# Villen-Lab/pyAscore

Hardware: AMD Instinct MI355X
Metric: PSMs/sec (Ascore.score) at 1/2/4/8 MI355X + HBM-roofline % (higher is better)
Workload: dtype f32/f64 scalar + i32 counts

## Files before the change

### pyascore_amd/csrc/common.h

```cpp
#ifndef PYA_COMMON_H
#define PYA_COMMON_H

#include <stdint.h>

#define PYA_WAVE 64
#define PYA_NTOP 10
#define PYA_NTOP_MAX 16
#define PYA_NO_MATCH 15
#define PYA_TABLE_PAD 4
#define PYA_MAX_L 64
#define PYA_MAX_TYPES 8
#define PYA_MAX_NL 8
#define PYA_FAST_NL 4
#define PYA_MAX_UNIQ_WIDE 48
#define PYA_MAX_NL_CANDS 44
#define PYA_MAX_UNIQ 16
#define PYA_MAX_LIST 2048
#define PYA_MAX_LUT_N 4096
#define PYA_MAX_PUSHED 128

#define PYA_ST_OK 0
#define PYA_ST_NO_BINS 1
#define PYA_ST_TOO_MANY_BINS 2
#define PYA_ST_LUT_RANGE 3
// ... 117 lines not shown
```

### pyascore_amd/csrc/fused_core.hip.h

```cpp
#ifndef PYA_FUSED_CORE_H
#define PYA_FUSED_CORE_H
#include "score_core.hip.h"
#include "localize_core.hip.h"

#define FUSED_ROUND 3

struct FusedLds {
    uint16_t *grid;
    uint4 *cum_lut;
    PeakEntry *peaks;
    float2 *resd;
    uint8_t *rkl;
    uint32_t *rec;
    float *wsl;
    float *mass_l;
    uint32_t *flag_l;
    uint8_t *site_pos;
    float *selm;
    unsigned char *sort_raw;
    PushedEntry *pushed;
    unsigned long long *site_alt;
    uint32_t *site_max, *site_tie, *n_pushed;
    float *sc;
    uint32_t *c_tr, *c_cnt;
// ... 8 lines not shown
__host__ __device__ static inline size_t fused_align16(size_t v) { return (v + 15) & ~(size_t)15; }
__host__ __device__ static inline size_t fused_sort_bytes(uint32_t n) {
    if (n <= 64) return ((size_t)n * 10 + 15) & ~(size_t)15;
    return (((size_t)n * 6 + 15) & ~(size_t)15) + ((size_t)n / 64 + 2) * 16 + 2 * 128 * 2;
}
__host__ __device__ static inline uint32_t fused_site_cap(uint32_t push_cap) {
    const uint32_t v = (push_cap + 3u) & ~3u;
    return v > 64u ? 64u : (v < 4u ? 4u : v);
}
__host__ __device__ static inline size_t fused_post_bytes(uint32_t n_cap, uint32_t push_cap, uint32_t ent_cap, uint32_t ndir,
                                                          bool multi_z) {
    return fused_align16(fused_sort_bytes(n_cap)) + (size_t)push_cap * 16 + (size_t)fused_site_cap(push_cap) * 16 + 16 +
           (size_t)(1 + FUSED_ROUND) * 40 + (size_t)FUSED_ROUND * (16 * ndir + 4 + 4) + 16 + 64 +
           (multi_z ? fused_align16((size_t)FUSED_ROUND * ndir * 2 * ent_cap * 4) +
                          fused_align16((size_t)FUSED_ROUND * ndir * 2 * ent_cap)
                    : 0);
}
__host__ __device__ static inline size_t fused_walk_bytes(uint32_t cap) {
    return 16 * 16 + ((size_t)cap + PYA_TABLE_PAD) * 8;
}
__host__ __device__ static inline size_t fused_kept_bytes(uint32_t n_cap, uint32_t stride, uint32_t pos_cap, uint32_t ent_cap,
                                                          uint32_t ndir) {
    return fused_align16(((size_t)pos_cap + 1) * 8) + fused_align16((size_t)ent_cap * stride) + (size_t)n_cap * 16 + 256 +
           fused_align16((size_t)pos_cap + 1) + (size_t)(1 + FUSED_ROUND) * ndir * ent_cap * 4;
}
__host__ __device__ static inline size_t fused_lds_bytes(uint32_t cap, uint32_t n_cap, uint32_t stride, uint32_t pos_cap,
                                                         uint32_t ent_cap, uint32_t push_cap, uint32_t ndir, bool multi_z) {
    const size_t walk = fused_walk_bytes(cap), post = fused_post_bytes(n_cap, push_cap, ent_cap, ndir, multi_z);
    return PYA_GRID_CELLS * 2 + fused_align16(walk > post ? walk : post) +
           fused_kept_bytes(n_cap, stride, pos_cap, ent_cap, ndir) + 16;
}

DEV FusedLds fused_carve(unsigned char *raw, uint32_t cap, uint32_t n_cap, uint32_t stride, uint32_t pos_cap,
                         uint32_t ent_cap, uint32_t push_cap, uint32_t ndir, bool multi_z) {
    FusedLds f;
    f.grid = (uint16_t *)raw;
    size_t o = PYA_GRID_CELLS * 2;
    f.cum_lut = (uint4 *)(raw + o);
    f.peaks = (PeakEntry *)(raw + o + 16 * 16);
// ... 14 lines not shown
    q += (size_t)(1 + FUSED_ROUND) * 40;
    f.c_tr = (uint32_t *)(raw + q);
    q += (size_t)FUSED_ROUND * ndir * 8;
    f.c_cnt = (uint32_t *)(raw + q);
    q += (size_t)FUSED_ROUND * ndir * 8;
    f.c_depth = (int32_t *)(raw + q);
    q += FUSED_ROUND * 4;
    f.c_site = (uint32_t *)(raw + q);
    q += FUSED_ROUND * 4;
    f.bad_tasks = (uint32_t *)(raw + q);
    q += 16;
    f.t_lo = (uint32_t *)(raw + q);
    f.t_off = f.t_lo + 8;
    q += 64;
    f.srt_v = (float *)(raw + q);
    q += fused_align16((size_t)FUSED_ROUND * ndir * 2 * ent_cap * 4);
    f.srt_h = (uint8_t *)(raw + q);
    const size_t walk = fused_walk_bytes(cap), post = fused_post_bytes(n_cap, push_cap, ent_cap, ndir, multi_z);
    o += fused_align16(walk > post ? walk : post);
    f.resd = (float2 *)(raw + o);
    o += fused_align16(((size_t)pos_cap + 1) * 8);
    f.rkl = (uint8_t *)(raw + o);
    o += fused_align16((size_t)ent_cap * stride);
    f.rec = (uint32_t *)(raw + o);
    o += (size_t)n_cap * 12;
    f.wsl = (float *)(raw + o);
    o += (size_t)n_cap * 4;
    f.mass_l = (float *)(raw + o);
    f.flag_l = (uint32_t *)(raw + o + 128);
    f.site_pos = (uint8_t *)(raw + o + 256);
    f.selm = (float *)(raw + o + 256 + fused_align16((size_t)pos_cap + 1));
    return f;
}


template <bool BZ>
DEV void walk_record_steps(const float2 *&rp, int rstride, StepBits &bits, float &running, const uint4 *lut, CumCounts &cum,
                           const PeakTable &tab, int zmax, double A, double B, uint8_t *&ro, int stride, int count) {
    for (int i = 0; i < count; i++, rp += rstride) {
        const float2 mm = *rp;
        running = (bits.next() ? mm.y : mm.x) + running;
        const double m = BZ ? (double)running + A : ((double)running + A) - B;
        for (int z = 1; z <= zmax; z++, ro += stride) {
            const Look k = look4(tab, charge_mz(m, z));
            int rk = k.best;
            if (k.more()) rk = look_rest(tab, k);
// ... 701 lines not shown
```

### pyascore_amd/csrc/host_internal.h

```cpp
#ifndef PYA_HOST_INTERNAL_H
#define PYA_HOST_INTERNAL_H
#include <hip/hip_runtime_api.h>

#include <algorithm>
#include <atomic>
#include <cmath>
#include <cstdarg>
#include <cstdio>
#include <cstdlib>
#include <chrono>
#include <cstring>
#include <condition_variable>
#include <map>
#include <memory>
#include <mutex>
#include <string>
#include <thread>
#include <unordered_map>
#include <vector>

#include "../../include/pyascore_hip.h"
#include "common.h"

void pya_score_table_extend(float mz_error, uint32_t n_top, uint32_t n_to, std::vector<float> &lut,
// ... 37 lines not shown
int pya_launch_score_big(const BatchDev *b, const uint32_t *d_ids, uint32_t n_ids, uint32_t cap, uint32_t pos_cap, uint32_t kc,
                         uint32_t inline_on, hipStream_t stream);
size_t pya_localize_recount_lds_bytes(uint32_t cap, uint32_t push_cap, uint32_t pos_cap, uint32_t pool_cap, uint32_t sb);
size_t pya_localize_hash_lds_bytes(uint32_t push_cap, uint32_t n_cap, uint32_t pos_cap, uint32_t sb, uint32_t vc, uint32_t hs,
                                   uint32_t pp, uint32_t max_k, uint32_t n_nl);
int pya_launch_localize_hash(const BatchDev *b, const uint32_t *d_ids, uint32_t n_ids, uint32_t push_cap, uint32_t n_cap,
                             uint32_t pos_cap, uint32_t pool_cap, uint32_t sb, uint32_t gtp, uint32_t vc, uint32_t hs, uint32_t pp,
                             uint32_t n_nl, hipStream_t stream);
int pya_launch_localize_recount(const BatchDev *b, const uint32_t *d_ids, uint32_t n_ids, uint32_t cap, uint32_t push_cap,
                                uint32_t pos_cap, uint32_t pool_cap, uint32_t sb, uint32_t gtp, uint32_t *d_redo_count, uint32_t *d_redo_ids, hipStream_t stream);
int pya_launch_score_big_list(const BatchDev *b, const uint32_t *d_count, const uint32_t *d_ids, uint32_t n_max, uint32_t cap,
                              uint32_t pos_cap, uint32_t kc, hipStream_t stream);
uint32_t pya_big_inline_max(void);
size_t pya_fused_lds_bytes(uint32_t cap, uint32_t n_cap, uint32_t stride, uint32_t pos_cap, uint32_t ent_cap, uint32_t push_cap,
                           uint32_t both, uint32_t multi_z);
int pya_launch_fused(const BatchDev *b, const uint32_t *d_ids, uint32_t n_ids, uint32_t cap, uint32_t n_cap,
                     uint32_t stride, uint32_t pos_cap, uint32_t ent_cap, uint32_t push_cap, uint32_t both,
                     uint32_t multi_z, uint32_t *d_redo_count, uint32_t *d_redo_ids, hipStream_t stream);
size_t pya_score_cnt_lds_bytes(uint32_t cap, uint32_t pos_cap, uint32_t kc, uint32_t k_cap, uint32_t n_cap);
int pya_launch_score_cnt(const BatchDev *b, const uint32_t *d_ids, uint32_t n_ids, uint32_t cap, uint32_t pos_cap, uint32_t kc, uint32_t k_cap,
                         uint32_t n_cap, hipStream_t stream);
size_t pya_score_cntg_lds_bytes(uint32_t cap, uint32_t pos_cap, uint32_t k_cap, uint32_t n_cap, uint32_t nl_cap);
int pya_launch_score_cntg(const BatchDev *b, const uint32_t *d_ids, uint32_t n_ids, uint32_t cap, uint32_t pos_cap, uint32_t k_cap, uint32_t n_cap,
                          uint32_t nl_cap, hipStream_t stream);
size_t pya_bin_global_scratch_bytes(uint32_t cap);
int pya_launch_bin_global(const BatchDev *b, const uint32_t *d_ids, uint32_t n_ids, unsigned char *d_scratch, uint64_t stride,
                          uint32_t cap, hipStream_t stream);
size_t pya_general_lds_bytes(uint32_t l_cap, uint32_t list_cap);
size_t pya_general_scratch_bytes(uint32_t n_cap, uint32_t push_cap);
int pya_launch_general(const BatchDev *b, const uint32_t *d_ids, uint32_t n_ids, unsigned char *d_scratch, const uint64_t *d_scratch_off,
                       uint32_t l_cap, uint32_t list_cap, hipStream_t stream);
int pya_launch_general_ambiguity(const BatchDev *b, uint32_t psm, uint32_t l_cap, uint32_t list_cap, uint64_t ref_bits,
                                 uint64_t oth_bits, const float *d_scores, uint32_t n_scores, float ref_ws, float oth_ws,
// ... 92 lines not shown
        case 'N': return 114.04293f;  case 'D': return 115.02694f;  case 'Q': return 128.05858f;
        case 'K': return 128.09496f;  case 'E': return 129.04259f;  case 'M': return 131.04049f;
        case 'H': return 137.05891f;  case 'F': return 147.06841f;  case 'U': return 150.95364f;
        case 'R': return 156.10111f;  case 'Y': return 163.06333f;  case 'W': return 186.07931f;
        case 'O': return 237.14773f;
    }
    return 0.f;
}


struct Knobs {
    bool no_plain = false, no_fused = false, no_big = false, no_tiny = false, no_prefix = false, no_chunks = false;
    bool no_upload_thread = false, one_peak_class = false, peak_classes = false, one_lds_class = false;
    bool host_timing = false, stamps = false, sort_room = false, no_big_inline = false;
    bool no_loc_hash = false, no_nodes = false, no_cnt = false;
    bool no_fork = false;
    bool slow_null_stream = false;
    uint32_t debug = 0;
    int64_t plain_min = 512, big_min_n = 1024, tiny_max = 64;
    int64_t bin_select_min = 640;
    int64_t bin_select_scap = 768;
    uint32_t sort_room_max = 1024;
    int sb = -1, gtp = -1, hash_pp = -1;
    int node_cap = -1;
    double chunk_mb = 0.;
    int64_t workspace_mb = 0;
};

void read_knobs(Knobs &k);
bool set_knob(Knobs &k, const char *key, const char *value);
// ... 212 lines not shown
    DevBuf<uint32_t> d_redo3;
    DevBuf<uint32_t> d_redo;
    Bucket buckets[kNumBuckets];
    struct IdList {
        uint32_t off, n, cap, ncls;
    };
    static bool any_ids(const std::vector<IdList> &lists) {
        bool any = false;
        for (const IdList &l : lists) any = any || l.n != 0;
        return any;
    }
    std::vector<uint32_t> bin_ids, score_ids, fused_ids, big_ids;
    std::vector<IdList> bin_lists, score_lists, big_lists;
    struct FusedLaunch {
        uint32_t off, n, cap, multi_z, n_cap, stride, pos_cap, ent_cap, push_cap;
    };
    std::vector<FusedLaunch> fused_launches;
    uint32_t n_fused_total = 0;
    std::vector<uint8_t> gen;
    std::vector<uint32_t> gen_ids;
    DevBuf<uint32_t> d_gen_ids;
    DevBuf<unsigned char> d_gen_scratch;
    uint32_t gen_l_cap = 1, gen_list_cap = 1;
    std::vector<uint64_t> gen_off;
    DevBuf<uint64_t> d_gen_off;
    std::vector<uint32_t> bigbin_ids;
    DevBuf<uint32_t> d_bigbin_ids;
    DevBuf<unsigned char> d_bigbin_scratch;
    uint32_t bigbin_cap = 32;
    size_t bigbin_stride = 0;
    std::vector<uint8_t> big;
    DevBuf<uint32_t> d_big_ids;
    uint32_t big_pos_cap = 1, big_k_max = 1;
// ... 119 lines not shown
```

### pyascore_amd/csrc/host_plan.cpp

```cpp
#include "host_internal.h"

int check_psm_shape(const pya_handle *h, uint64_t i, int64_t P, int64_t L, int32_t k, int32_t z, const uint8_t *pep,
                    const uint32_t *aux_pos, int64_t n_aux, uint32_t *ns, char *msg) {
    const unsigned long long iu = i;
    auto say = [msg](int code, const char *fmt, auto... args) {
        std::snprintf(msg, kPsmMsg, fmt, args...);
        return code;
    };
    if (P <= 0) return say(PYA_ERR_PSM, "PSM %llu: empty spectrum", iu);
    if (P > PYA_MAX_PEAKS) return say(PYA_ERR_LIMIT, "PSM %llu: %lld peaks exceed the limit of %d", iu, (long long)P, PYA_MAX_PEAKS);
    if (L < 1 || L > PYA_MAX_PEPTIDE_LEN)
        return say(L < 1 ? PYA_ERR_PSM : PYA_ERR_LIMIT, "PSM %llu: peptide length %lld outside 1..%d", iu, (long long)L, PYA_MAX_PEPTIDE_LEN);
    if (k < 0) return say(PYA_ERR_PSM, "PSM %llu: negative n_of_mod", iu);
    if (z < 1 || z > PYA_MAX_CHARGE)
        return say(z < 1 ? PYA_ERR_PSM : PYA_ERR_LIMIT, "PSM %llu: max_fragment_charge %d outside 1..%d", iu, z, PYA_MAX_CHARGE);
    if (n_aux < 0) return say(PYA_ERR_ARG, "PSM %llu: aux_off is not monotone", iu);
    uint32_t cnt = 0;
    int64_t bad_j = -1, bad_a = -1;
    for (int64_t j = 0; j < L; j++) {
        if (!h->is_residue[pep[j]] && bad_j < 0) bad_j = j;
        if (h->letter_modifiable((char)pep[j], (size_t)j, (size_t)L)) cnt++;
    }
    for (int64_t a = 0; a < n_aux; a++)
        if (aux_pos[a] > (uint32_t)L && bad_a < 0) bad_a = a;
// ... 24 lines not shown
    std::vector<uint8_t> bad;
    std::vector<uint32_t> caps;
    std::vector<uint8_t> pcls;

    PlanBuild(pya_handle *h_, const pya_batch *b_, const IoReq *io_, uint32_t flags_, pya_plan *p_)
        : h(h_), b(b_), io(io_), flags(flags_), p(p_), n(b_->n_psm) {
        const DevConfig &c = h->cfg;
        const Knobs &kn = h->kn;
        has_aux = b->aux_off && b->aux_pos && b->aux_mass;
        plain_on = c.n_nl == 0 && !(flags & PYA_FLAG_KEEP) && !kn.no_plain && n >= (uint64_t)kn.plain_min;
        both_dirs = c.n_fwd > 0 && c.n_fwd < c.n_types;
        fused_on = plain_on && plain_types(c) && !kn.no_fused;
        big_on = c.n_nl == 0 && both_dirs && c.n_fwd == 1 && c.n_types == 2 && h->mz_error <= 0.49f && !kn.no_big;
        big_inline_ok = big_on && plain_on && !kn.no_big_inline;
        big_inline_max = pya_big_inline_max();
    }
};

struct Lap {
    bool on;
    std::chrono::steady_clock::time_point t0 = std::chrono::steady_clock::now();
    void operator()(const char *what) {
        if (!on) return;
        auto t1 = std::chrono::steady_clock::now();
        std::fprintf(stderr, "[pya plan] %-14s %8.3f ms\n", what, std::chrono::duration<double, std::milli>(t1 - t0).count());
        t0 = t1;
    }
};

int copy_meta(PlanBuild &B) {
// ... 240 lines not shown
            const size_t at = (size_t)(q * (double)(n - 1));
            size_t acc = 0;
            uint32_t v = 0;
            for (; v < hist.size(); v++) {
                acc += hist[v];
                if (acc > at) break;
            }
            caps.push_back((v + 31u) & ~31u);
        }
    }
    if (!caps.empty() && p->peak_cap < 2 * caps[0] && !h->kn.peak_classes) caps.clear();
    caps.push_back(p->peak_cap);
    std::sort(caps.begin(), caps.end());
    caps.erase(std::unique(caps.begin(), caps.end()), caps.end());
    const size_t nc = caps.size();
    std::vector<uint32_t> cnt_bin(nc, 0), cnt_score(nc * kNumBuckets, 0), cnt_big(nc, 0);
    B.pcls.resize(n);
    for (uint64_t i = 0; i < n; i++) {
        if (p->pre_status[i]) continue;
        const uint32_t P = (uint32_t)(p->peak_off[i + 1] - p->peak_off[i]);
        if (P > PYA_FAST_PEAKS) continue;
        size_t c = 0;
        while (caps[c] < P) c++;
        B.pcls[i] = (uint8_t)c;
        cnt_bin[c]++;
        if (p->fused[i] || p->gen[i]) continue;
        if (p->big[i]) cnt_big[c]++;
        else cnt_score[p->ncls[i] * nc + c]++;
    }
    uint32_t n_bin = 0, n_score = 0, n_big = 0;
    for (size_t c = 0; c < nc; c++) {
        p->bin_lists.push_back({n_bin, 0u, caps[c], 0u});
        n_bin += cnt_bin[c];
    }
    for (size_t g = 0; g < nc * kNumBuckets; g++) {
        p->score_lists.push_back({n_score, 0u, caps[g % nc], (uint32_t)(g / nc)});
        n_score += cnt_score[g];
    }
    for (size_t c = 0; c < nc; c++) {
        p->big_lists.push_back({n_big, 0u, caps[c], 0u});
        n_big += cnt_big[c];
    }
    p->bin_ids.resize(n_bin);
    p->score_ids.resize(n_score);
    p->big_ids.resize(n_big);
    for (uint64_t i = 0; i < n; i++) {
        if (p->pre_status[i]) continue;
        if (p->peak_off[i + 1] - p->peak_off[i] > PYA_FAST_PEAKS) continue;
        pya_plan::IdList &bl = p->bin_lists[B.pcls[i]];
        p->bin_ids[bl.off + bl.n++] = (uint32_t)i;
        if (p->fused[i] || p->gen[i]) continue;
        pya_plan::IdList &sl = p->big[i] ? p->big_lists[B.pcls[i]] : p->score_lists[p->ncls[i] * nc + B.pcls[i]];
        (p->big[i] ? p->big_ids : p->score_ids)[sl.off + sl.n++] = (uint32_t)i;
    }
}

struct FusedItem {
    uint32_t id, group;
    size_t need;
    uint32_t n_cap, pos, ent, push;
};

void sort_fused_items(std::vector<FusedItem> &items) {
    std::vector<std::pair<uint64_t, uint32_t>> keys;
    keys.reserve(256);
// ... 53 lines not shown
        size_t g1 = g0;
        while (g1 < items.size() && items[g1].group == items[g0].group) g1++;
        std::vector<size_t> cuts{g0};
        if (g1 - g0 >= 8192 && !B.h->kn.one_lds_class) {
            const size_t need_max = items[g1 - 1].need;
            for (double q : {0.5, 0.85}) {
                const size_t at = g0 + (size_t)(q * (double)(g1 - g0));
                size_t cut = at;
                while (cut < g1 && items[cut].need == items[at].need) cut++;
                if (cut < g1 && cut > cuts.back() && items[at].need * 5 <= need_max * 4) cuts.push_back(cut);
            }
        }
        cuts.push_back(g1);
        for (size_t c = 0; c + 1 < cuts.size(); c++) {
            pya_plan::FusedLaunch fl = {(uint32_t)cuts[c], (uint32_t)(cuts[c + 1] - cuts[c]), B.caps[items[g0].group / 2],
                                        items[g0].group & 1u, 4, 4, 1, 1, 8};
            for (size_t t = cuts[c]; t < cuts[c + 1]; t++) {
                fl.n_cap = std::max(fl.n_cap, items[t].n_cap);
                fl.pos_cap = std::max(fl.pos_cap, items[t].pos);
                fl.ent_cap = std::max(fl.ent_cap, items[t].ent);
                fl.push_cap = std::max(fl.push_cap, items[t].push);
                p->fused_ids[t] = items[t].id;
            }
            fl.stride = ndir * fl.n_cap + 4;
            p->fused_launches.push_back(fl);
        }
        g0 = g1;
    }
}

void pack_descriptors(PlanBuild &B) {
// ... 291 lines not shown
```

### pyascore_amd/csrc/host_run.cpp

```cpp
#include "host_internal.h"

namespace {

struct ScoreRoute {
    enum Kind { kCountNodes, kCountNodesGeneral, kSignatures } kind;
    uint32_t prefix, compact, kc, node_cap, node_cols, res_cap, nl_cap;
};

ScoreRoute pick_score_route(const pya_handle *h, const Bucket &bk, uint32_t ncls, uint32_t peak_cap) {
    const DevConfig &c = h->cfg;
    ScoreRoute r = {ScoreRoute::kSignatures, score_prefix(h, bk.n_cap), score_compact(c, bk.z_max), 8u, 0u, 0u, 0u, nl_cap(c)};
    const bool general = general_settings(c);
    const bool cnt_ok = h->mz_error <= 0.49f && bk.k_max + 1u <= 31u && bk.ns_max <= 32u && !h->kn.no_cnt && !(h->kn.debug & 0x8000u);
    if (ncls >= 1 && !general && c.n_fwd == 1 && c.n_types == 2 && bk.z_max == 1 && cnt_ok) {
        while (r.kc < bk.k_max + 1u) r.kc <<= 1;
        if (pya_score_cnt_lds_bytes(peak_cap, bk.pos_cap, r.kc, bk.k_max, bk.ns_max) <= 64u * 1024u) {
            r.kind = ScoreRoute::kCountNodes;
            return r;
        }
    }
    if (general && cnt_ok && pya_score_cntg_lds_bytes(peak_cap, bk.pos_cap, bk.k_max, bk.ns_max, r.nl_cap) <= 64u * 1024u) {
        r.kind = ScoreRoute::kCountNodesGeneral;
        return r;
    }
// ... 45 lines not shown
    *done = true;
    return PYA_OK;
}

int run_binning(pya_plan *p, const BatchDev &d, hipStream_t st) {
    pya_handle *h = p->h;
    int e = 0;
    for (const pya_plan::IdList &l : p->bin_lists) {
        const uint32_t scap = (uint32_t)std::min<int64_t>(std::max<int64_t>(h->kn.bin_select_scap, 64), 4096) & ~31u;
        if ((int64_t)l.cap > h->kn.bin_select_min)
            e = pya_launch_bin_select(&d, p->d_bin_ids.p + l.off, l.n, scap, st);
        else
            e = pya_launch_bin(&d, p->d_bin_ids.p + l.off, l.n, l.cap, st);
        if (e) return h->hip_fail((hipError_t)e, "bin_spectra launch");
    }
    e = pya_launch_bin_exact(&d, (uint32_t)p->n_psm, p->peak_cap, st);
    if (e) return h->hip_fail((hipError_t)e, "bin_spectra (exact) launch");
    e = pya_launch_bin_global(&d, p->d_bigbin_ids.p, (uint32_t)p->bigbin_ids.size(), p->d_bigbin_scratch.p, p->bigbin_stride, p->bigbin_cap, st);
    if (e) return h->hip_fail((hipError_t)e, "bin_spectra (global) launch");
    return PYA_OK;
}

int run_fused_family(pya_plan *p, const BatchDev &d, hipStream_t fs) {
    pya_handle *h = p->h;
    const Bucket &fb = p->fusedb;
    for (const pya_plan::FusedLaunch &l : p->fused_launches) {
        int fe = pya_launch_fused(&d, p->d_fused_ids.p + l.off, l.n, l.cap, l.n_cap, l.stride, l.pos_cap, l.ent_cap, l.push_cap,
                                  p->fused_both, l.multi_z, d.redo4_count, d.redo4_ids, fs);
        if (fe) return h->hip_fail((hipError_t)fe, "score_localize launch");
    }
    int fe = pya_launch_localize_redo(&d, d.redo4_count, d.redo4_ids, p->n_fused_total, fb.push_cap(), fb.n_cap,
                                      fb.pos_cap, fb.pool_cap(), fb.sb(), fb.gtp(), fs);
    if (fe) return h->hip_fail((hipError_t)fe, "localize (hand-over) launch");
    return PYA_OK;
}

int run_scoring(pya_plan *p, const BatchDev &d, hipStream_t st) {
    pya_handle *h = p->h;
    int e = 0;
    for (const pya_plan::IdList &l : p->score_lists) {
        const Bucket &bk = p->buckets[l.ncls];
        const uint32_t *ids = p->d_score_ids.p + l.off;
        const ScoreRoute r = pick_score_route(h, bk, l.ncls, l.cap);
        switch (r.kind) {
            case ScoreRoute::kCountNodes:
                e = pya_launch_score_cnt(&d, ids, l.n, l.cap, bk.pos_cap, r.kc, bk.k_max, bk.ns_max, st);
                if (e) return h->hip_fail((hipError_t)e, "score_cnt launch");
// ... 52 lines not shown
        else
            e = pya_launch_localize(&d, general_ids, n_general, bk.push_cap(), bk.n_cap, bk.pos_cap, bk.pool_cap(), bk.sb(),
                                    bk.gtp(), 0u, 1u, st);
        if (e) return h->hip_fail((hipError_t)e, "localize launch");
    }
    return PYA_OK;
}

int run_general(pya_plan *p, const BatchDev &d, hipStream_t st) {
    int e = pya_launch_general(&d, p->d_gen_ids.p, (uint32_t)p->gen_ids.size(), p->d_gen_scratch.p, p->d_gen_off.p, p->gen_l_cap,
                               p->gen_list_cap, st);
    if (e) return p->h->hip_fail((hipError_t)e, "general kernel launch");
    return PYA_OK;
}

int run_behind_binning(pya_plan *p, const BatchDev &d, hipStream_t st, const RunMarks &mark) {
    pya_handle *h = p->h;
    int rc;
    if (mark.alias) mark.alias[5] = 0;
    if (p->fork) {
        HIPCHK(h, hipStreamWaitEvent(p->side, p->ev_fork, 0));
        if (mark.ev) {
            mark.alias[5] = 1;
            HIPCHK(h, hipEventRecord(mark.ev[5], p->side));
        }
        if ((rc = run_fused_family(p, d, p->side))) return rc;
        if (mark.ev) HIPCHK(h, hipEventRecord(mark.ev[6], p->side));
    }
    if ((rc = run_scoring(p, d, st))) return rc;
    if ((rc = mark(2, pya_plan::any_ids(p->score_lists) || pya_plan::any_ids(p->big_lists)))) return rc;
    const bool fused_here = p->n_fused_total != 0 && !p->fork;
    if (fused_here && (rc = run_fused_family(p, d, st))) return rc;
    if ((rc = mark(3, fused_here))) return rc;
    const bool big_inline = p->big_inline && !p->bigloc.ids.empty();
    if (big_inline && (rc = run_big_inline(p, d, st))) return rc;
    if ((rc = run_localize(p, d, st))) return rc;
    if (!p->gen_ids.empty() && (rc = run_general(p, d, st))) return rc;
    if (mark.ev) {
        bool loc = big_inline || !p->gen_ids.empty();
        for (const Bucket &bk : p->buckets) loc = loc || !bk.ids.empty();
        if ((rc = mark(4, loc))) return rc;
        p->ev_runs++;
        if (p->ev_runs - p->ev_read > pya_plan::kEvRing) p->ev_read = p->ev_runs - pya_plan::kEvRing;
// ... 24 lines not shown
    d.n_sig_out = o->n_sig;
    d.ascores = o->ascores;
    d.alt_mask = o->alt_mask;
    d.max_k = o->max_k;
    bool tiny = false;
    int rc = run_tiny(p, d, st, &tiny);
    if (rc) return rc;
    if (!tiny) {
        const bool timing = p->flags & PYA_FLAG_TIMING;
        const RunMarks mark = {h, st, timing ? p->ev_set(p->ev_runs) : nullptr, timing ? p->ev_alias(p->ev_runs) : nullptr};
        if ((rc = mark(0, true))) return rc;
        uint32_t *cnt = p->d_redo.p + 8 * (p->n_runs & 1u);
        d.redo_count = cnt;
        d.redo4_count = cnt + 1;
        d.zero_next = p->d_redo.p + 8 * ((p->n_runs + 1u) & 1u);
        if (p->n_runs == 0 || !pya_plan::any_ids(p->bin_lists)) HIPCHK(h, hipMemsetAsync(p->d_redo.p, 0, 16 * sizeof(uint32_t), st));
        p->n_runs++;
        if ((rc = run_binning(p, d, st))) return rc;
        if ((rc = mark(1, true))) return rc;
        if (!p->fork) {
            if ((rc = run_behind_binning(p, d, st, mark))) return rc;
        } else {
            HIPCHK(h, hipEventRecord(p->ev_fork, st));
            rc = run_behind_binning(p, d, st, mark);
            hipError_t ej = hipEventRecord(p->ev_join, p->side);
            if (ej == hipSuccess) ej = hipStreamWaitEvent(st, p->ev_join, 0);
            if (ej != hipSuccess && !rc) rc = h->hip_fail(ej, "joining the side stream");
        }
    }
    p->last_stream = st;
    p->ran = true;
    p->dev = d;
    return rc;
}

namespace {
int add_run_intervals(pya_plan *p, uint64_t r0, uint64_t r1, double ms[4]) {
    pya_handle *h = p->h;
    HIPCHK(h, hipEventSynchronize(p->ev_set(r1 - 1)[p->ev_alias(r1 - 1)[4]]));
// ... 100 lines not shown
```

### pyascore_amd/csrc/host_tables.cpp

```cpp
#include "host_internal.h"

static void read_env(Knobs &k) {
    auto flag = [](const char *n) { return std::getenv(n) != nullptr; };
    k.host_timing = flag("PYA_HOST_TIMING");
    k.stamps = flag("PYA_STAMPS");
    k.chunk_mb = 0.;
    if (const char *e = std::getenv("PYA_CHUNK_MB")) k.chunk_mb = std::max(1.0, std::atof(e));
    const char *w = std::getenv("PYA_WORKSPACE_MB");
    k.workspace_mb = w ? (int64_t)std::atoll(w) : 0;
}

void read_knobs(Knobs &k) {
    k = Knobs();
    read_env(k);
}

bool set_knob(Knobs &k, const char *key, const char *value) {
    const Knobs dflt;
    const std::string name(key ? key : "");
    const bool on = value != nullptr;
    auto num = [&](int64_t d) { return on ? (int64_t)std::strtoll(value, nullptr, 0) : d; };
    struct { const char *n; bool Knobs::*m; } flags[] = {
        {"PYA_NO_PLAIN", &Knobs::no_plain}, {"PYA_NO_FUSED", &Knobs::no_fused}, {"PYA_NO_BIG", &Knobs::no_big},
        {"PYA_NO_TINY", &Knobs::no_tiny}, {"PYA_NO_PREFIX", &Knobs::no_prefix}, {"PYA_NO_CHUNKS", &Knobs::no_chunks},
        {"PYA_NO_UPLOAD_THREAD", &Knobs::no_upload_thread}, {"PYA_ONE_PEAK_CLASS", &Knobs::one_peak_class},
        {"PYA_PEAK_CLASSES", &Knobs::peak_classes}, {"PYA_ONE_LDS_CLASS", &Knobs::one_lds_class},
        {"PYA_SORT_ROOM", &Knobs::sort_room}, {"PYA_NO_BIG_INLINE", &Knobs::no_big_inline},
        {"PYA_NO_LOC_HASH", &Knobs::no_loc_hash}, {"PYA_NO_CNT", &Knobs::no_cnt}, {"PYA_NO_NODES", &Knobs::no_nodes},
        {"PYA_HOST_TIMING", &Knobs::host_timing}, {"PYA_STAMPS", &Knobs::stamps},
        {"PYA_SLOW_NULL_STREAM", &Knobs::slow_null_stream}, {"PYA_NO_FORK", &Knobs::no_fork},
    };
    bool known = false;
    for (auto &f : flags)
        if (name == f.n) {
            k.*(f.m) = on;
            known = true;
        }
    if (name == "PYA_DEBUG") k.debug = (uint32_t)num(0), known = true;
    else if (name == "PYA_PLAIN_MIN") k.plain_min = num(dflt.plain_min), known = true;
    else if (name == "PYA_BIG_MIN_N") k.big_min_n = num(dflt.big_min_n), known = true;
    else if (name == "PYA_BIN_SELECT_MIN") k.bin_select_min = num(dflt.bin_select_min), known = true;
    else if (name == "PYA_BIN_SELECT_SCAP") k.bin_select_scap = num(dflt.bin_select_scap), known = true;
    else if (name == "PYA_TINY_MAX") k.tiny_max = num(dflt.tiny_max), known = true;
    else if (name == "PYA_SORT_ROOM_MAX") k.sort_room_max = (uint32_t)num(dflt.sort_room_max), known = true;
    else if (name == "PYA_SB") k.sb = (int)num(-1), known = true;
// ... 229 lines not shown
```

### pyascore_amd/csrc/score_localize.hip

```cpp
#include "fused_core.hip.h"

#ifndef FUSED_WAVES
#define FUSED_WAVES 6
#endif

template <bool BOTH, bool ZM, bool WIDE = false>
__global__ __launch_bounds__(64, FUSED_WAVES) void pya_score_localize_kernel(
    BatchDev b, const uint32_t *psm_ids, uint32_t n_ids, uint32_t cap, uint32_t n_cap, uint32_t stride, uint32_t pos_cap,
    uint32_t ent_cap, uint32_t push_cap, uint32_t *redo_count, uint32_t *redo_ids) {
    extern __shared__ __attribute__((aligned(16))) unsigned char lds_raw[];
    if (blockIdx.x >= n_ids) return;
    const uint32_t psm = psm_ids[xcd_slot(blockIdx.x, n_ids)];
    const bool declined = fused_body<BOTH, ZM, WIDE>(b, psm, lds_raw, cap, n_cap, stride, pos_cap, ent_cap, push_cap);
    if (declined && lane_id() == 0) redo_ids[atomicAdd(redo_count, 1u)] = psm;
}

extern "C" size_t pya_fused_lds_bytes(uint32_t cap, uint32_t n_cap, uint32_t stride, uint32_t pos_cap, uint32_t ent_cap,
                                      uint32_t push_cap, uint32_t both, uint32_t multi_z) {
    return fused_lds_bytes(cap, n_cap, stride, pos_cap, ent_cap, push_cap, both ? 2u : 1u, multi_z != 0);
}

extern "C" int pya_launch_fused(const BatchDev *b, const uint32_t *d_ids, uint32_t n_ids, uint32_t cap, uint32_t n_cap,
                                uint32_t stride, uint32_t pos_cap, uint32_t ent_cap, uint32_t push_cap, uint32_t both,
                                uint32_t multi_z, uint32_t *d_redo_count, uint32_t *d_redo_ids, hipStream_t stream) {
    if (n_ids == 0) return 0;
    const size_t lds = fused_lds_bytes(cap, n_cap, stride, pos_cap, ent_cap, push_cap, both ? 2u : 1u, multi_z != 0);
#define PYA_FUSED_LAUNCH(B, Z, W)                                                                                          \
    do {                                                                                                                   \
        hipError_t e = PYA_ENSURE_MAX_LDS((pya_score_localize_kernel<B, Z, W>));                                           \
        if (e != hipSuccess) return (int)e;                                                                                \
        hipLaunchKernelGGL((pya_score_localize_kernel<B, Z, W>), dim3(n_ids), dim3(64), lds, stream, *b, d_ids, n_ids, cap, \
                           n_cap, stride, pos_cap, ent_cap, push_cap, d_redo_count, d_redo_ids);                           \
    } while (0)
    const bool wide = both && n_cap > 32u;
    if (both && multi_z && wide) PYA_FUSED_LAUNCH(true, true, true);
    else if (both && wide) PYA_FUSED_LAUNCH(true, false, true);
    else if (both && multi_z) PYA_FUSED_LAUNCH(true, true, false);
    else if (both) PYA_FUSED_LAUNCH(true, false, false);
    else if (multi_z) PYA_FUSED_LAUNCH(false, true, false);
    else PYA_FUSED_LAUNCH(false, false, false);
#undef PYA_FUSED_LAUNCH
    return (int)hipGetLastError();
}
```

### pyascore_amd/csrc/tiny_batch.hip

```cpp
#include "bin_core.hip.h"
#include "score_core.hip.h"
#include "localize_body.hip.h"
#include "fused_core.hip.h"

__global__ __launch_bounds__(64) void pya_tiny_batch_kernel(BatchDev b, uint32_t n_psm, uint32_t cap, uint32_t prefix,
                                                            uint32_t with_nl, uint32_t compact, uint32_t push_cap,
                                                            uint32_t pos_cap, uint32_t pool_cap, uint32_t sb,
                                                            uint32_t gtp) {
    extern __shared__ __attribute__((aligned(16))) unsigned char lds_raw[];
    const uint32_t psm = blockIdx.x;
    if (psm >= n_psm) return;
    {
        const float *r_mz;
        const uint8_t *r_rank;
        int status;
        int R = bin_core<false>(b, psm, lds_raw, cap, &r_mz, &r_rank, &status);
        if (R == PYA_BIN_REDO) {
            wave_lds_sync();
            R = bin_core<true>(b, psm, lds_raw, cap, &r_mz, &r_rank, &status);
        }
        bin_store(b, psm, R, status, r_mz, r_rank);
    }
    __threadfence();
    wave_lds_sync();
// ... 11 lines not shown
    size_t s = score_lds_bytes(cap, prefix, with_nl, prefix ? compact : 0u);
    size_t l = localize_lds_bytes(push_cap, n_cap, pos_cap, pool_cap, sb);
    a = a > s ? a : s;
    return a > l ? a : l;
}

extern "C" int pya_launch_tiny(const BatchDev *b, uint32_t n_psm, uint32_t cap, uint32_t prefix, uint32_t with_nl,
                               uint32_t compact, uint32_t push_cap, uint32_t n_cap, uint32_t pos_cap,
                               uint32_t pool_cap, uint32_t sb, uint32_t gtp, hipStream_t stream) {
    if (n_psm == 0) return 0;
    const size_t lds = pya_tiny_lds_bytes(cap, prefix, with_nl, compact, push_cap, n_cap, pos_cap, pool_cap, sb);
    hipError_t e = PYA_ENSURE_MAX_LDS(pya_tiny_batch_kernel);
    if (e != hipSuccess) return (int)e;
    hipLaunchKernelGGL(pya_tiny_batch_kernel, dim3(n_psm), dim3(64), lds, stream, *b, n_psm, cap, prefix, with_nl,
                       compact, push_cap, pos_cap, pool_cap, sb, gtp);
    return (int)hipGetLastError();
}


template <bool ZM>
__global__ __launch_bounds__(64) void pya_one_kernel(BatchDev b, OneMeta m, uint32_t cap, uint32_t prefix, uint32_t with_nl,
                                                     uint32_t compact, uint32_t push_cap, uint32_t pos_cap, uint32_t pool_cap,
                                                     uint32_t sb, uint32_t gtp, uint32_t use_fused, uint32_t f_n_cap,
                                                     uint32_t f_stride, uint32_t f_ent_cap, uint32_t f_push_cap,
                                                     int32_t *host_status, uint32_t *host_flag) {
    extern __shared__ __attribute__((aligned(16))) unsigned char lds_raw[];
    const int lane = lane_id();
    const uint64_t tk0 = __builtin_amdgcn_s_memrealtime(), cy0 = __builtin_amdgcn_s_memtime();
    BinPre pre;
    bin_preload(b.mz, b.inten, m.n_peaks, &pre);
// ... 102 lines not shown
```

Before: 204.0 million.

## Fuse binning into score-localize kernel for single-chain fused batches

Result: faster. 209.1 million, median of 6 (+2.5%).

```diff
diff --git a/pyascore_amd/csrc/common.h b/pyascore_amd/csrc/common.h
--- a/pyascore_amd/csrc/common.h
+++ b/pyascore_amd/csrc/common.h
@@ -7,6 +7,7 @@
 #define PYA_NTOP 10
 #define PYA_NTOP_MAX 16
 #define PYA_NO_MATCH 15
+#define PYA_REDO_REBIN 0x80000000u
 #define PYA_TABLE_PAD 4
 #define PYA_MAX_L 64
 #define PYA_MAX_TYPES 8
diff --git a/pyascore_amd/csrc/fused_core.hip.h b/pyascore_amd/csrc/fused_core.hip.h
--- a/pyascore_amd/csrc/fused_core.hip.h
+++ b/pyascore_amd/csrc/fused_core.hip.h
@@ -46,15 +46,20 @@
            (size_t)(1 + FUSED_ROUND) * 40 + (size_t)FUSED_ROUND * (16 * ndir + 4 + 4) + 16 + 64 +
            (multi_z ? fused_align16((size_t)FUSED_ROUND * ndir * 2 * ent_cap * 4) +
                           fused_align16((size_t)FUSED_ROUND * ndir * 2 * ent_cap)
-                    : 0);
+                    : 0) +
+           fused_align16((size_t)(1 + FUSED_ROUND) * ndir * ent_cap * 4);
+}
+__host__ __device__ static inline size_t fused_rec_bytes(uint32_t n_cap) {
+    return (size_t)n_cap * 16 > 256 ? (size_t)n_cap * 16 : 256;
 }
 __host__ __device__ static inline size_t fused_walk_bytes(uint32_t cap) {
     return 16 * 16 + ((size_t)cap + PYA_TABLE_PAD) * 8;
 }
 __host__ __device__ static inline size_t fused_kept_bytes(uint32_t n_cap, uint32_t stride, uint32_t pos_cap, uint32_t ent_cap,
                                                           uint32_t ndir) {
-    return fused_align16(((size_t)pos_cap + 1) * 8) + fused_align16((size_t)ent_cap * stride) + (size_t)n_cap * 16 + 256 +
-           fused_align16((size_t)pos_cap + 1) + (size_t)(1 + FUSED_ROUND) * ndir * ent_cap * 4;
+    (void)ndir;
+    return fused_align16(((size_t)pos_cap + 1) * 8) + fused_align16((size_t)ent_cap * stride) + fused_rec_bytes(n_cap) +
+           fused_align16((size_t)pos_cap + 1);
 }
 __host__ __device__ static inline size_t fused_lds_bytes(uint32_t cap, uint32_t n_cap, uint32_t stride, uint32_t pos_cap,
                                                          uint32_t ent_cap, uint32_t push_cap, uint32_t ndir, bool multi_z) {
@@ -99,8 +104,9 @@
     f.t_off = f.t_lo + 8;
     q += 64;
     f.srt_v = (float *)(raw + q);
-    q += fused_align16((size_t)FUSED_ROUND * ndir * 2 * ent_cap * 4);
-    f.srt_h = (uint8_t *)(raw + q);
+    f.srt_h = (uint8_t *)(raw + q + fused_align16((size_t)FUSED_ROUND * ndir * 2 * ent_cap * 4));
+    if (multi_z) q += fused_align16((size_t)FUSED_ROUND * ndir * 2 * ent_cap * 4) + fused_align16((size_t)FUSED_ROUND * ndir * 2 * ent_cap);
+    f.selm = (float *)(raw + q);
     const size_t walk = fused_walk_bytes(cap), post = fused_post_bytes(n_cap, push_cap, ent_cap, ndir, multi_z);
     o += fused_align16(walk > post ? walk : post);
     f.resd = (float2 *)(raw + o);
@@ -108,13 +114,11 @@
     f.rkl = (uint8_t *)(raw + o);
     o += fused_align16((size_t)ent_cap * stride);
     f.rec = (uint32_t *)(raw + o);
-    o += (size_t)n_cap * 12;
-    f.wsl = (float *)(raw + o);
-    o += (size_t)n_cap * 4;
+    f.wsl = (float *)(raw + o + (size_t)n_cap * 12);
     f.mass_l = (float *)(raw + o);
     f.flag_l = (uint32_t *)(raw + o + 128);
-    f.site_pos = (uint8_t *)(raw + o + 256);
-    f.selm = (float *)(raw + o + 256 + fused_align16((size_t)pos_cap + 1));
+    o += fused_rec_bytes(n_cap);
+    f.site_pos = (uint8_t *)(raw + o);
     return f;
 }
 
diff --git a/pyascore_amd/csrc/host_internal.h b/pyascore_amd/csrc/host_internal.h
--- a/pyascore_amd/csrc/host_internal.h
+++ b/pyascore_amd/csrc/host_internal.h
@@ -75,9 +75,16 @@
 uint32_t pya_big_inline_max(void);
 size_t pya_fused_lds_bytes(uint32_t cap, uint32_t n_cap, uint32_t stride, uint32_t pos_cap, uint32_t ent_cap, uint32_t push_cap,
                            uint32_t both, uint32_t multi_z);
+size_t pya_merged_lds_bytes(uint32_t cap, uint32_t n_cap, uint32_t stride, uint32_t pos_cap, uint32_t ent_cap, uint32_t push_cap,
+                            uint32_t both, uint32_t multi_z);
 int pya_launch_fused(const BatchDev *b, const uint32_t *d_ids, uint32_t n_ids, uint32_t cap, uint32_t n_cap,
                      uint32_t stride, uint32_t pos_cap, uint32_t ent_cap, uint32_t push_cap, uint32_t both,
-                     uint32_t multi_z, uint32_t *d_redo_count, uint32_t *d_redo_ids, hipStream_t stream);
+                     uint32_t multi_z, uint32_t merged, uint32_t *d_redo_count, uint32_t *d_redo_ids, hipStream_t stream);
+size_t pya_score_localize_list_lds_bytes(uint32_t cap, uint32_t push_cap, uint32_t n_cap, uint32_t pos_cap, uint32_t pool_cap,
+                                         uint32_t sb);
+int pya_launch_score_localize_list(const BatchDev *b, const uint32_t *d_count, const uint32_t *d_ids, uint32_t n_max, uint32_t cap,
+                                   uint32_t push_cap, uint32_t n_cap, uint32_t pos_cap, uint32_t pool_cap, uint32_t sb,
+                                   uint32_t gtp, hipStream_t stream);
 size_t pya_score_cnt_lds_bytes(uint32_t cap, uint32_t pos_cap, uint32_t kc, uint32_t k_cap, uint32_t n_cap);
 int pya_launch_score_cnt(const BatchDev *b, const uint32_t *d_ids, uint32_t n_ids, uint32_t cap, uint32_t pos_cap, uint32_t kc, uint32_t k_cap,
                          uint32_t n_cap, hipStream_t stream);
@@ -200,6 +207,7 @@
     bool no_upload_thread = false, one_peak_class = false, peak_classes = false, one_lds_class = false;
     bool host_timing = false, stamps = false, sort_room = false, no_big_inline = false;
     bool no_loc_hash = false, no_nodes = false, no_cnt = false;
+    bool no_merge = false;
     bool no_fork = false;
     bool slow_null_stream = false;
     uint32_t debug = 0;
@@ -442,9 +450,11 @@
     std::vector<IdList> bin_lists, score_lists, big_lists;
     struct FusedLaunch {
         uint32_t off, n, cap, multi_z, n_cap, stride, pos_cap, ent_cap, push_cap;
+        uint32_t merged;
     };
     std::vector<FusedLaunch> fused_launches;
     uint32_t n_fused_total = 0;
+    uint32_t merged_cap = 0;
     std::vector<uint8_t> gen;
     std::vector<uint32_t> gen_ids;
     DevBuf<uint32_t> d_gen_ids;
diff --git a/pyascore_amd/csrc/host_plan.cpp b/pyascore_amd/csrc/host_plan.cpp
--- a/pyascore_amd/csrc/host_plan.cpp
+++ b/pyascore_amd/csrc/host_plan.cpp
@@ -62,6 +62,11 @@
         big_on = c.n_nl == 0 && both_dirs && c.n_fwd == 1 && c.n_types == 2 && h->mz_error <= 0.49f && !kn.no_big;
         big_inline_ok = big_on && plain_on && !kn.no_big_inline;
         big_inline_max = pya_big_inline_max();
+    }
+    bool single_chain = false;
+    bool merges(uint32_t cap) const {
+        return fused_on && single_chain && !h->kn.no_merge && (int64_t)cap <= h->kn.bin_select_min &&
+               pya_bin_lds_bytes(cap) <= 64u * 1024u;
     }
 };
 
@@ -332,6 +337,8 @@
     std::sort(caps.begin(), caps.end());
     caps.erase(std::unique(caps.begin(), caps.end()), caps.end());
     const size_t nc = caps.size();
+    B.single_chain = true;
+    for (uint64_t i = 0; i < n; i++) B.single_chain = B.single_chain && (p->pre_status[i] || p->fused[i]);
     std::vector<uint32_t> cnt_bin(nc, 0), cnt_score(nc * kNumBuckets, 0), cnt_big(nc, 0);
     B.pcls.resize(n);
     for (uint64_t i = 0; i < n; i++) {
@@ -341,7 +348,7 @@
         size_t c = 0;
         while (caps[c] < P) c++;
         B.pcls[i] = (uint8_t)c;
-        cnt_bin[c]++;
+        if (!(p->fused[i] && B.merges(caps[c]))) cnt_bin[c]++;
         if (p->fused[i] || p->gen[i]) continue;
         if (p->big[i]) cnt_big[c]++;
         else cnt_score[p->ncls[i] * nc + c]++;
@@ -366,7 +373,7 @@
         if (p->pre_status[i]) continue;
         if (p->peak_off[i + 1] - p->peak_off[i] > PYA_FAST_PEAKS) continue;
         pya_plan::IdList &bl = p->bin_lists[B.pcls[i]];
-        p->bin_ids[bl.off + bl.n++] = (uint32_t)i;
+        if (!(p->fused[i] && B.merges(bl.cap))) p->bin_ids[bl.off + bl.n++] = (uint32_t)i;
         if (p->fused[i] || p->gen[i]) continue;
         pya_plan::IdList &sl = p->big[i] ? p->big_lists[B.pcls[i]] : p->score_lists[p->ncls[i] * nc + B.pcls[i]];
         (p->big[i] ? p->big_ids : p->score_ids)[sl.off + sl.n++] = (uint32_t)i;
@@ -450,7 +457,9 @@
         cuts.push_back(g1);
         for (size_t c = 0; c + 1 < cuts.size(); c++) {
             pya_plan::FusedLaunch fl = {(uint32_t)cuts[c], (uint32_t)(cuts[c + 1] - cuts[c]), B.caps[items[g0].group / 2],
-                                        items[g0].group & 1u, 4, 4, 1, 1, 8};
+                                        items[g0].group & 1u, 4, 4, 1, 1, 8, 0};
+            fl.merged = B.merges(fl.cap) ? 1u : 0u;
+            if (fl.merged) p->merged_cap = std::max(p->merged_cap, fl.cap);
             for (size_t t = cuts[c]; t < cuts[c + 1]; t++) {
                 fl.n_cap = std::max(fl.n_cap, items[t].n_cap);
                 fl.pos_cap = std::max(fl.pos_cap, items[t].pos);
diff --git a/pyascore_amd/csrc/host_run.cpp b/pyascore_amd/csrc/host_run.cpp
--- a/pyascore_amd/csrc/host_run.cpp
+++ b/pyascore_amd/csrc/host_run.cpp
@@ -83,7 +83,7 @@
             e = pya_launch_bin(&d, p->d_bin_ids.p + l.off, l.n, l.cap, st);
         if (e) return h->hip_fail((hipError_t)e, "bin_spectra launch");
     }
-    e = pya_launch_bin_exact(&d, (uint32_t)p->n_psm, p->peak_cap, st);
+    if (pya_plan::any_ids(p->bin_lists)) e = pya_launch_bin_exact(&d, (uint32_t)p->n_psm, p->peak_cap, st);
     if (e) return h->hip_fail((hipError_t)e, "bin_spectra (exact) launch");
     e = pya_launch_bin_global(&d, p->d_bigbin_ids.p, (uint32_t)p->bigbin_ids.size(), p->d_bigbin_scratch.p, p->bigbin_stride, p->bigbin_cap, st);
     if (e) return h->hip_fail((hipError_t)e, "bin_spectra (global) launch");
@@ -95,11 +95,13 @@
     const Bucket &fb = p->fusedb;
     for (const pya_plan::FusedLaunch &l : p->fused_launches) {
         int fe = pya_launch_fused(&d, p->d_fused_ids.p + l.off, l.n, l.cap, l.n_cap, l.stride, l.pos_cap, l.ent_cap, l.push_cap,
-                                  p->fused_both, l.multi_z, d.redo4_count, d.redo4_ids, fs);
+                                  p->fused_both, l.multi_z, l.merged, d.redo4_count, d.redo4_ids, fs);
         if (fe) return h->hip_fail((hipError_t)fe, "score_localize launch");
     }
-    int fe = pya_launch_localize_redo(&d, d.redo4_count, d.redo4_ids, p->n_fused_total, fb.push_cap(), fb.n_cap,
-                                      fb.pos_cap, fb.pool_cap(), fb.sb(), fb.gtp(), fs);
+    int fe = p->merged_cap ? pya_launch_score_localize_list(&d, d.redo4_count, d.redo4_ids, p->n_fused_total, p->merged_cap, fb.push_cap(),
+                                                            fb.n_cap, fb.pos_cap, fb.pool_cap(), fb.sb(), fb.gtp(), fs)
+                           : pya_launch_localize_redo(&d, d.redo4_count, d.redo4_ids, p->n_fused_total, fb.push_cap(), fb.n_cap,
+                                                      fb.pos_cap, fb.pool_cap(), fb.sb(), fb.gtp(), fs);
     if (fe) return h->hip_fail((hipError_t)fe, "localize (hand-over) launch");
     return PYA_OK;
 }
@@ -182,19 +184,23 @@
     return PYA_OK;
 }
 
+int fork_fused_family(pya_plan *p, const BatchDev &d, hipStream_t st, const RunMarks &mark) {
+    pya_handle *h = p->h;
+    int rc;
+    HIPCHK(h, hipEventRecord(p->ev_fork, st));
+    HIPCHK(h, hipStreamWaitEvent(p->side, p->ev_fork, 0));
+    if (mark.ev) {
+        mark.alias[5] = 1;
+        HIPCHK(h, hipEventRecord(mark.ev[5], p->side));
+    }
+    if ((rc = run_fused_family(p, d, p->side))) return rc;
+    if (mark.ev) HIPCHK(h, hipEventRecord(mark.ev[6], p->side));
+    return PYA_OK;
+}
+
 int run_behind_binning(pya_plan *p, const BatchDev &d, hipStream_t st, const RunMarks &mark) {
-    pya_handle *h = p->h;
     int rc;
-    if (mark.alias) mark.alias[5] = 0;
-    if (p->fork) {
-        HIPCHK(h, hipStreamWaitEvent(p->side, p->ev_fork, 0));
-        if (mark.ev) {
-            mark.alias[5] = 1;
-            HIPCHK(h, hipEventRecord(mark.ev[5], p->side));
-        }
-        if ((rc = run_fused_family(p, d, p->side))) return rc;
-        if (mark.ev) HIPCHK(h, hipEventRecord(mark.ev[6], p->side));
-    }
+    if (p->fork && (rc = fork_fused_family(p, d, st, mark))) return rc;
     if ((rc = run_scoring(p, d, st))) return rc;
     if ((rc = mark(2, pya_plan::any_ids(p->score_lists) || pya_plan::any_ids(p->big_lists)))) return rc;
     const bool fused_here = p->n_fused_total != 0 && !p->fork;
@@ -249,15 +255,20 @@
         d.redo_count = cnt;
         d.redo4_count = cnt + 1;
         d.zero_next = p->d_redo.p + 8 * ((p->n_runs + 1u) & 1u);
-        if (p->n_runs == 0 || !pya_plan::any_ids(p->bin_lists)) HIPCHK(h, hipMemsetAsync(p->d_redo.p, 0, 16 * sizeof(uint32_t), st));
+        if (p->n_runs == 0 || !(pya_plan::any_ids(p->bin_lists) || p->merged_cap))
+            HIPCHK(h, hipMemsetAsync(p->d_redo.p, 0, 16 * sizeof(uint32_t), st));
         p->n_runs++;
-        if ((rc = run_binning(p, d, st))) return rc;
-        if ((rc = mark(1, true))) return rc;
+        if (mark.alias) mark.alias[5] = 0;
+        auto rest = [&]() -> int {
+            int r;
+            if ((r = run_binning(p, d, st))) return r;
+            if ((r = mark(1, true))) return r;
+            return run_behind_binning(p, d, st, mark);
+        };
         if (!p->fork) {
-            if ((rc = run_behind_binning(p, d, st, mark))) return rc;
+            if ((rc = rest())) return rc;
         } else {
-            HIPCHK(h, hipEventRecord(p->ev_fork, st));
-            rc = run_behind_binning(p, d, st, mark);
+            rc = rest();
             hipError_t ej = hipEventRecord(p->ev_join, p->side);
             if (ej == hipSuccess) ej = hipStreamWaitEvent(st, p->ev_join, 0);
             if (ej != hipSuccess && !rc) rc = h->hip_fail(ej, "joining the side stream");
diff --git a/pyascore_amd/csrc/host_tables.cpp b/pyascore_amd/csrc/host_tables.cpp
--- a/pyascore_amd/csrc/host_tables.cpp
+++ b/pyascore_amd/csrc/host_tables.cpp
@@ -29,6 +29,7 @@
         {"PYA_NO_LOC_HASH", &Knobs::no_loc_hash}, {"PYA_NO_CNT", &Knobs::no_cnt}, {"PYA_NO_NODES", &Knobs::no_nodes},
         {"PYA_HOST_TIMING", &Knobs::host_timing}, {"PYA_STAMPS", &Knobs::stamps},
         {"PYA_SLOW_NULL_STREAM", &Knobs::slow_null_stream}, {"PYA_NO_FORK", &Knobs::no_fork},
+        {"PYA_NO_MERGE", &Knobs::no_merge},
     };
     bool known = false;
     for (auto &f : flags)
diff --git a/pyascore_amd/csrc/score_localize.hip b/pyascore_amd/csrc/score_localize.hip
--- a/pyascore_amd/csrc/score_localize.hip
+++ b/pyascore_amd/csrc/score_localize.hip
@@ -1,3 +1,4 @@
+#include "bin_core.hip.h"
 #include "fused_core.hip.h"
 
 #ifndef FUSED_WAVES
@@ -15,22 +16,58 @@
     if (declined && lane_id() == 0) redo_ids[atomicAdd(redo_count, 1u)] = psm;
 }
 
+template <bool BOTH, bool ZM, bool WIDE = false>
+__global__ __launch_bounds__(64, FUSED_WAVES) void pya_bin_score_localize_kernel(
+    BatchDev b, const uint32_t *psm_ids, uint32_t n_ids, uint32_t cap, uint32_t n_cap, uint32_t stride, uint32_t pos_cap,
+    uint32_t ent_cap, uint32_t push_cap, uint32_t *redo_count, uint32_t *redo_ids) {
+    extern __shared__ __attribute__((aligned(16))) unsigned char lds_raw[];
+    if (blockIdx.x == 0 && threadIdx.x < 3 && b.zero_next) b.zero_next[threadIdx.x] = 0u;
+    if (blockIdx.x >= n_ids) return;
+    const uint32_t psm = psm_ids[xcd_slot(blockIdx.x, n_ids)];
+    const float *r_mz;
+    const uint8_t *r_rank;
+    int status;
+    const int R = bin_fast<false>(b, psm, lds_raw, cap, &r_mz, &r_rank, &status);
+    bool declined = R == PYA_BIN_REDO || R > FUSED_LOCAL_CHUNKS * 64 - PYA_TABLE_PAD;
+    if (!declined) {
+        if (R < 0) bin_store(b, psm, R, status, r_mz, r_rank);
+        else if (lane_id() == 0) b.status[psm] = PYA_ST_OK;
+        const LocalTable lt = {r_mz, r_rank, R < 0 ? 0 : R, R < 0 ? status : PYA_ST_OK};
+        declined = fused_body<BOTH, ZM, WIDE>(b, psm, lds_raw, cap, n_cap, stride, pos_cap, ent_cap, push_cap, &lt);
+    }
+    if (declined && lane_id() == 0) redo_ids[atomicAdd(redo_count, 1u)] = psm | PYA_REDO_REBIN;
+}
+
 extern "C" size_t pya_fused_lds_bytes(uint32_t cap, uint32_t n_cap, uint32_t stride, uint32_t pos_cap, uint32_t ent_cap,
                                       uint32_t push_cap, uint32_t both, uint32_t multi_z) {
     return fused_lds_bytes(cap, n_cap, stride, pos_cap, ent_cap, push_cap, both ? 2u : 1u, multi_z != 0);
 }
 
+extern "C" size_t pya_merged_lds_bytes(uint32_t cap, uint32_t n_cap, uint32_t stride, uint32_t pos_cap, uint32_t ent_cap,
+                                       uint32_t push_cap, uint32_t both, uint32_t multi_z) {
+    const size_t f = fused_lds_bytes(cap, n_cap, stride, pos_cap, ent_cap, push_cap, both ? 2u : 1u, multi_z != 0);
+    const size_t a = PYA_BIN_FAST_BYTES(cap);
+    return a > f ? a : f;
+}
+
 extern "C" int pya_launch_fused(const BatchDev *b, const uint32_t *d_ids, uint32_t n_ids, uint32_t cap, uint32_t n_cap,
                                 uint32_t stride, uint32_t pos_cap, uint32_t ent_cap, uint32_t push_cap, uint32_t both,
-                                uint32_t multi_z, uint32_t *d_redo_count, uint32_t *d_redo_ids, hipStream_t stream) {
+                                uint32_t multi_z, uint32_t merged, uint32_t *d_redo_count, uint32_t *d_redo_ids,
+                                hipStream_t stream) {
     if (n_ids == 0) return 0;
-    const size_t lds = fused_lds_bytes(cap, n_cap, stride, pos_cap, ent_cap, push_cap, both ? 2u : 1u, multi_z != 0);
+    const size_t lds = merged ? pya_merged_lds_bytes(cap, n_cap, stride, pos_cap, ent_cap, push_cap, both, multi_z)
+                              : fused_lds_bytes(cap, n_cap, stride, pos_cap, ent_cap, push_cap, both ? 2u : 1u, multi_z != 0);
+#define PYA_FUSED_LAUNCH_OF(KERNEL, B, Z, W)                                                                               \
+    do {                                                                                                                   \
+        hipError_t e = PYA_ENSURE_MAX_LDS((KERNEL<B, Z, W>));                                                              \
+        if (e != hipSuccess) return (int)e;                                                                                \
+        hipLaunchKernelGGL((KERNEL<B, Z, W>), dim3(n_ids), dim3(64), lds, stream, *b, d_ids, n_ids, cap, n_cap, stride,    \
+                           pos_cap, ent_cap, push_cap, d_redo_count, d_redo_ids);                                          \
+    } while (0)
 #define PYA_FUSED_LAUNCH(B, Z, W)                                                                                          \
     do {                                                                                                                   \
-        hipError_t e = PYA_ENSURE_MAX_LDS((pya_score_localize_kernel<B, Z, W>));                                           \
-        if (e != hipSuccess) return (int)e;                                                                                \
-        hipLaunchKernelGGL((pya_score_localize_kernel<B, Z, W>), dim3(n_ids), dim3(64), lds, stream, *b, d_ids, n_ids, cap, \
-                           n_cap, stride, pos_cap, ent_cap, push_cap, d_redo_count, d_redo_ids);                           \
+        if (merged) PYA_FUSED_LAUNCH_OF(pya_bin_score_localize_kernel, B, Z, W);                                           \
+        else PYA_FUSED_LAUNCH_OF(pya_score_localize_kernel, B, Z, W);                                                      \
     } while (0)
     const bool wide = both && n_cap > 32u;
     if (both && multi_z && wide) PYA_FUSED_LAUNCH(true, true, true);
@@ -40,5 +77,6 @@
     else if (multi_z) PYA_FUSED_LAUNCH(false, true, false);
     else PYA_FUSED_LAUNCH(false, false, false);
 #undef PYA_FUSED_LAUNCH
+#undef PYA_FUSED_LAUNCH_OF
     return (int)hipGetLastError();
 }
diff --git a/pyascore_amd/csrc/tiny_batch.hip b/pyascore_amd/csrc/tiny_batch.hip
--- a/pyascore_amd/csrc/tiny_batch.hip
+++ b/pyascore_amd/csrc/tiny_batch.hip
@@ -49,6 +49,48 @@
     if (e != hipSuccess) return (int)e;
     hipLaunchKernelGGL(pya_tiny_batch_kernel, dim3(n_psm), dim3(64), lds, stream, *b, n_psm, cap, prefix, with_nl,
                        compact, push_cap, pos_cap, pool_cap, sb, gtp);
+    return (int)hipGetLastError();
+}
+
+__global__ __launch_bounds__(64) void pya_score_localize_list_kernel(BatchDev b, const uint32_t *count, const uint32_t *ids,
+                                                                     uint32_t cap, uint32_t push_cap, uint32_t pos_cap,
+                                                                     uint32_t pool_cap, uint32_t sb, uint32_t gtp) {
+    extern __shared__ __attribute__((aligned(16))) unsigned char lds_raw[];
+    const uint32_t n = *count;
+    for (uint32_t k = blockIdx.x; k < n; k += gridDim.x) {
+        const uint32_t entry = ids[k], psm = entry & ~PYA_REDO_REBIN;
+        if (entry & PYA_REDO_REBIN) {
+            const float *r_mz;
+            const uint8_t *r_rank;
+            int status;
+            const int R = bin_core<true>(b, psm, lds_raw, cap, &r_mz, &r_rank, &status);
+            bin_store(b, psm, R, status, r_mz, r_rank);
+            __threadfence();
+            wave_lds_sync();
+            score_body<false>(b, psm, lds_raw, cap, 0u, 0u);
+            __threadfence();
+            wave_lds_sync();
+        }
+        localize_body<false>(b, psm, lds_raw, push_cap, pos_cap, pool_cap, sb, gtp);
+        wave_lds_sync();
+    }
+}
+
+extern "C" size_t pya_score_localize_list_lds_bytes(uint32_t cap, uint32_t push_cap, uint32_t n_cap, uint32_t pos_cap,
+                                                    uint32_t pool_cap, uint32_t sb) {
+    return pya_tiny_lds_bytes(cap, 0u, 0u, 0u, push_cap, n_cap, pos_cap, pool_cap, sb);
+}
+
+extern "C" int pya_launch_score_localize_list(const BatchDev *b, const uint32_t *d_count, const uint32_t *d_ids, uint32_t n_max,
+                                              uint32_t cap, uint32_t push_cap, uint32_t n_cap, uint32_t pos_cap,
+                                              uint32_t pool_cap, uint32_t sb, uint32_t gtp, hipStream_t stream) {
+    if (n_max == 0) return 0;
+    const size_t lds = pya_score_localize_list_lds_bytes(cap, push_cap, n_cap, pos_cap, pool_cap, sb);
+    hipError_t e = PYA_ENSURE_MAX_LDS(pya_score_localize_list_kernel);
+    if (e != hipSuccess) return (int)e;
+    const uint32_t grid = n_max < 8192u ? n_max : 8192u;
+    hipLaunchKernelGGL(pya_score_localize_list_kernel, dim3(grid), dim3(64), lds, stream, *b, d_count, d_ids, cap, push_cap,
+                       pos_cap, pool_cap, sb, gtp);
     return (int)hipGetLastError();
 }
 
```
